# jhauret/vibravox

Hardware: AMD Instinct MI355X
Metric: EBEN train-step audio-seconds/sec (gen+disc) (higher is better)
Workload: dtype bf16

## Files before the change

### include/eben_hip.h

```cpp
#ifndef EBEN_HIP_H
#define EBEN_HIP_H

#include <stddef.h>
#include <stdint.h>

#if defined(EBEN_BUILDING)
#define EBEN_API __attribute__((visibility("default")))
#else
#define EBEN_API
#endif

#ifdef __cplusplus
extern "C" {
#endif

#define EBEN_OK 0
#define EBEN_EINVAL (-1)
#define EBEN_EWORKSPACE (-2)
#define EBEN_EUNSUPPORTED (-3)

#define EBEN_PAD_ZERO 0
#define EBEN_PAD_REFLECT 1

#define EBEN_MATH_F32 0
// ... 30 lines not shown
  int32_t rows, cols;
} EbenWnScaleItem;
typedef struct EbenWnBwdItem {
  const float* slabs;
  const float* g; const float* v; const float* norm;
  float* dg; float* dv; float* dbias;
  int64_t slab_stride;
  int32_t nslab, rows, cols, row_stride;
  int32_t col_perm_k, pad_;
} EbenWnBwdItem;
EBEN_API int eben_wn_scale_multi(const EbenWnScaleItem* items, int n, void* stream);
EBEN_API int eben_wn_bwd_multi(const EbenWnBwdItem* items, int n, void* stream);

EBEN_API size_t eben_conv1d_packed_floats(const EbenConv1dDesc* d, int which);
typedef struct EbenPackJob {
  EbenConv1dDesc desc;
  const float* v; const float* scale;
  float* wp_fwd; float* wp_bwd;
} EbenPackJob;
EBEN_API int eben_conv1d_pack_multi(const EbenPackJob* jobs, int n, void* stream);
#define EBEN_CONV_ROUTE_NONE 0
#define EBEN_CONV_ROUTE_TAP1 1
#define EBEN_CONV_ROUTE_TAP2 2
#define EBEN_CONV_ROUTE_THIN 3
#define EBEN_CONV_ROUTE_TAP3 4
#define EBEN_CONV_ROUTE_GC 5
#define EBEN_CONV_ROUTE_TAP4 6
EBEN_API int eben_conv1d_kernel_generation(const EbenConv1dDesc* d, int which);
#define EBEN_VARIANT_TAP3 1
#define EBEN_VARIANT_THIN_BL 2
#define EBEN_VARIANT_TAP4 3
#define EBEN_VARIANT_GC 4
EBEN_API int eben_conv1d_variant(const EbenConv1dDesc* d, int which, int mask_on_load, int* out, int n);
EBEN_API int eben_conv1d_variant_f32(const EbenConv1dDesc* d, int which, int mask_on_load, int* out, int n);
EBEN_API int eben_conv1d_pack(const EbenConv1dDesc* d, const float* v, const float* scale, float* wp_fwd, float* wp_bwd, void* stream);
EBEN_API int eben_conv1d_fwd(const EbenConv1dDesc* d, const float* x, const float* wp_fwd, const float* bias,
                    const float* residual, float* y, void* stream);
EBEN_API int eben_conv1d_fwd_res(const EbenConv1dDesc* d, const float* x, const float* wp_fwd, const float* bias,
                        const float* residual, float res_slope, float* y, void* stream);
EBEN_API size_t eben_conv1d_bwd_dx_workspace(const EbenConv1dDesc* d);
EBEN_API size_t eben_conv1d_bwd_dw_workspace(const EbenConv1dDesc* d, int* nslab, int* row_stride);
EBEN_API int eben_conv1d_bwd_dx(const EbenConv1dDesc* d, const float* dy, const float* y, const float* wp_bwd,
                       const float* x, float* dx, int accumulate, void* workspace, size_t ws_bytes, void* stream);
EBEN_API int eben_conv1d_bwd_dx_res(const EbenConv1dDesc* d, const float* dy, const float* y, const float* wp_bwd, const float* x,
                           const float* res_pre, const float* res_post, float* dx, void* workspace, size_t ws_bytes, void* stream);
EBEN_API int eben_conv1d_bwd_dx_ex(const EbenConv1dDesc* d, const float* g, const float* wp_bwd, const float* res, int res_rows,
                          const float* mask, float mask_slope, int seg, const int* seg_map, float* dx, void* stream);
EBEN_API int eben_conv1d_bwd_dx_fm(const EbenConv1dDesc* d, const float* g, const float* wp_bwd, const float* ref, int fm_rows,
                          const float* fm_sums, float fm_gs, const float* mask, float mask_slope, int seg, const int* seg_map,
                          float* dx, void* stream);
EBEN_API int eben_conv1d_bwd_dw(const EbenConv1dDesc* d, const float* dy, const float* y, const float* x, int has_bias,
                       float* slabs, size_t ws_bytes, void* stream);
#define EBEN_DW_ROUTE_TINY 0
#define EBEN_DW_ROUTE_ONE_ROW 1
#define EBEN_DW_ROUTE_DW3 2
#define EBEN_DW_ROUTE_DW2 3
#define EBEN_DW_ROUTE_FALLBACK 4
EBEN_API int eben_conv1d_bwd_dw_variant(const EbenConv1dDesc* d, int* out, int n);
EBEN_API int eben_conv1d_bwd_dw_f32_variant(const EbenConv1dDesc* d, int* out, int n);

EBEN_API int eben_bl_from_f32(const float* x, int batch, int channels, int length, void* hi, void* lo , void* stream);
EBEN_API int eben_bl_to_f32(const void* hi, const void* lo , int batch, int channels, int length, float* x, void* stream);
EBEN_API int eben_bl_conv1d_fwd(const EbenConv1dDesc* d, const void* x_hi, const void* x_lo, const float* wp_fwd, const float* bias,
                       void* y_hi, void* y_lo, void* stream);
EBEN_API int eben_bl_conv1d_bwd_dx(const EbenConv1dDesc* d, const void* g_hi, const float* wp_bwd, const void* act_hi, const void* act_lo,
                          float mask_slope, int seg, const int* seg_map, int fm_rows, int ref_row_offset, const float* fm_sums,
// ... 388 lines not shown
```

### vibravox_amd/_lib.py

```python
from __future__ import annotations

import ctypes
import os
from ctypes import POINTER, c_char_p, c_float, c_int, c_int32, c_int64, c_size_t, c_void_p
from typing import Optional

import torch

_HERE = os.path.dirname(os.path.abspath(__file__))
LIB_PATH = os.path.join(_HERE, "lib", "libeben_hip.so")


class EbenError(RuntimeError):
    pass


class EbenConv1dDesc(ctypes.Structure):
    _fields_ = [
        ("batch", c_int32),
        ("c_in", c_int32),
        ("c_out", c_int32),
        ("l_in", c_int32),
        ("l_out", c_int32),
        ("ksize", c_int32),
# ... 107 lines not shown
    _fields_ = [("band", c_void_p), ("first", c_void_p), ("orig", c_int32), ("nw", c_int32), ("width", c_int32), ("W", c_int32)]


class EbenResampleClip(ctypes.Structure):
    _fields_ = [("src_offset", c_int64), ("t_in", c_int32), ("band", c_int32), ("dst_row", c_int32), ("reserved", c_int32)]


class EbenVocoderClip(ctypes.Structure):
    _fields_ = [("rate", ctypes.c_double), ("frames_out", c_int32), ("col_out", c_int32)]


class EbenOlaClip(ctypes.Structure):
    _fields_ = [("dst_offset", c_int64), ("col", c_int32), ("frames_out", c_int32), ("len_stretch", c_int32), ("valid", c_int32)]


class EbenMaskClip(ctypes.Structure):
    _fields_ = [("row", c_int32), ("first", c_int32), ("count", c_int32)]


_P = c_void_p
_D = POINTER(EbenConv1dDesc)

SIGNATURES = {
    "eben_last_error": (c_char_p, []),
    "eben_version": (c_int, []),
    "eben_device_info": (c_int, [ctypes.c_char_p, c_size_t]),
    "eben_wn_scale": (c_int, [_P, _P, c_int, c_int, _P, _P, _P]),
    "eben_wn_bwd": (c_int, [_P, c_int, c_size_t, c_int, c_int, c_int, _P, _P, _P, _P, _P, _P, _P]),
    "eben_wn_scale_multi": (c_int, [POINTER(EbenWnScaleItem), c_int, _P]),
    "eben_wn_bwd_multi": (c_int, [POINTER(EbenWnBwdItem), c_int, _P]),
    "eben_conv1d_packed_floats": (c_size_t, [_D, c_int]),
    "eben_conv1d_kernel_generation": (c_int, [_D, c_int]),
    "eben_conv1d_variant": (c_int, [_D, c_int, c_int, POINTER(c_int), c_int]),
    "eben_conv1d_variant_f32": (c_int, [_D, c_int, c_int, POINTER(c_int), c_int]),
    "eben_conv1d_pack": (c_int, [_D, _P, _P, _P, _P, _P]),
    "eben_conv1d_pack_multi": (c_int, [POINTER(EbenPackJob), c_int, _P]),
    "eben_conv1d_fwd": (c_int, [_D, _P, _P, _P, _P, _P, _P]),
    "eben_conv1d_fwd_res": (c_int, [_D, _P, _P, _P, _P, c_float, _P, _P]),
    "eben_conv1d_bwd_dx_res": (c_int, [_D, _P, _P, _P, _P, _P, _P, _P, _P, c_size_t, _P]),
    "eben_conv1d_bwd_dx_workspace": (c_size_t, [_D]),
    "eben_conv1d_bwd_dw_workspace": (c_size_t, [_D, POINTER(c_int), POINTER(c_int)]),
    "eben_conv1d_bwd_dx": (c_int, [_D, _P, _P, _P, _P, _P, c_int, _P, c_size_t, _P]),
    "eben_conv1d_bwd_dx_ex": (c_int, [_D, _P, _P, _P, c_int, _P, c_float, c_int, POINTER(c_int), _P, _P]),
    "eben_conv1d_bwd_dx_fm": (c_int, [_D, _P, _P, _P, c_int, _P, c_float, _P, c_float, c_int, POINTER(c_int), _P, _P]),
    "eben_conv1d_bwd_dw": (c_int, [_D, _P, _P, _P, c_int, _P, c_size_t, _P]),
    "eben_conv1d_bwd_dw_variant": (c_int, [_D, POINTER(c_int), c_int]),
    "eben_conv1d_bwd_dw_f32_variant": (c_int, [_D, POINTER(c_int), c_int]),
    "eben_bl_from_f32": (c_int, [_P, c_int, c_int, c_int, _P, _P, _P]),
    "eben_bl_to_f32": (c_int, [_P, _P, c_int, c_int, c_int, _P, _P]),
    "eben_bl_conv1d_fwd": (c_int, [_D, _P, _P, _P, _P, _P, _P, _P]),
    "eben_bl_conv1d_bwd_dx": (c_int, [_D, _P, _P, _P, _P, c_float, c_int, POINTER(c_int), c_int, c_int, _P, c_float, _P, _P, _P]),
    "eben_bl_dx_pr_desc": (c_int, [_D, _D]),
    "eben_bl_dx_pr_weights": (c_int, [_D, _P, _P, _P, _P]),
    "eben_bl_conv1d_bwd_dx_pr": (c_int, [_D, _P, _P, _P, _P, c_float, c_int, POINTER(c_int), c_int, c_int, _P, c_float, _P, _P, _P]),
    "eben_bl_conv1d_bwd_dx_c": (c_int, [_D, _P, _P, _P, _P, _P, c_float, c_int, POINTER(c_int), c_int, c_int, _P, c_float, _P, _P, _P]),
    "eben_bl_conv1d_bwd_dx_pr_c": (c_int, [_D, _P, _P, _P, _P, _P, c_float, c_int, POINTER(c_int), c_int, c_int, _P, c_float, _P, _P, _P]),
    "eben_bl_conv1d_bwd_dw_workspace": (c_size_t, [_D, POINTER(c_int), POINTER(c_int), POINTER(c_int)]),
    "eben_bl_conv1d_bwd_dw": (c_int, [_D, _P, _P, c_int, _P, c_size_t, _P]),
    "eben_bl_conv1d_bwd_dw_multi": (c_int, [POINTER(_D), POINTER(_P), POINTER(_P), c_int, POINTER(_P), POINTER(c_size_t), c_int, _P]),
    "eben_bl_conv1d_bwd_dw_variant": (c_int, [_D, POINTER(c_int), c_int]),
    "eben_bl_head_fwd": (c_int, [POINTER(EbenBlHeadJob), c_int, c_int, _P]),
    "eben_bl_head_dx": (c_int, [POINTER(EbenBlHeadJob), c_int, c_int, _P, _P]),
    "eben_bl_head_dw_workspace": (c_size_t, [POINTER(EbenBlHeadJob), c_int, POINTER(c_int), POINTER(c_int)]),
    "eben_bl_head_dw": (c_int, [POINTER(EbenBlHeadJob), c_int, _P, c_size_t, _P]),
    "eben_bl_tail_fwd": (c_int, [_P, _P, c_int, c_int, c_int, c_int, c_int, _P, _P, _P, c_float, _P, _P]),
    "eben_bl_tail_dx": (c_int, [_P, c_int, c_int, c_int, c_int, c_int, _P, _P, _P, _P, c_float, c_int, POINTER(c_int), c_int, c_int, _P, c_float,
# ... 191 lines not shown
```

### vibravox_amd/csrc/conv1d.hip

```cpp
#include "common.h"
#include "tap3.h"

#include <cstdlib>

namespace eben {

int canon_from_desc(const EbenConv1dDesc* d, Canon* c) {
  EBEN_REQUIRE(d != nullptr, "null conv descriptor");
  EBEN_REQUIRE(d->batch > 0 && d->c_in > 0 && d->c_out > 0 && d->l_in > 0 && d->l_out > 0, "non-positive conv dims");
  EBEN_REQUIRE(d->ksize > 0 && d->stride > 0 && d->dilation > 0 && d->groups > 0, "non-positive conv params");
  EBEN_REQUIRE(d->c_in % d->groups == 0 && d->c_out % d->groups == 0, "channels not divisible by groups");
  EBEN_REQUIRE(d->stride <= 1024 && d->pad_l >= 0 && d->pad_r >= 0, "bad stride / padding");
  c->B = d->batch; c->k = d->ksize; c->s = d->stride; c->d = d->dilation; c->g = d->groups;
  c->pl = d->pad_l; c->pr = d->pad_r;
  const int math = d->math & ~EBEN_LAYOUT_BL;
  EBEN_REQUIRE(math >= EBEN_MATH_F32 && math <= EBEN_MATH_BF16X6, "unknown math mode %d", d->math);
  c->bl = (d->math & EBEN_LAYOUT_BL) != 0;
  EBEN_REQUIRE(!c->bl || math == EBEN_MATH_BF16 || math == EBEN_MATH_BF16X3, "the bundle layout carries EBEN_MATH_BF16 / EBEN_MATH_BF16X3 only");
  c->bf16 = math != EBEN_MATH_F32;
  c->np = math == EBEN_MATH_BF16X3 ? 2 : (math == EBEN_MATH_BF16X6 ? 3 : 1);
  c->xsplit_dir = math == EBEN_MATH_BF16X2 ? (d->transposed ? 1 : 0) : -1;
  if (!d->transposed) {
    c->Cin = d->c_in; c->Cout = d->c_out; c->Lin = d->l_in; c->Lout = d->l_out;
    c->reflect = d->pad_mode == EBEN_PAD_REFLECT;
// ... 87 lines not shown

extern "C" size_t eben_conv1d_packed_floats(const EbenConv1dDesc* d, int which) {
  Canon c;
  if (canon_from_desc(d, &c) != EBEN_OK) return 0;
  const ConvRoute r = conv_route(c, d->transposed, which);
  return kConvFamilies[r.family].packed_floats(c, r.dir);
}

extern "C" int eben_conv1d_kernel_generation(const EbenConv1dDesc* d, int which) {
  Canon c;
  if (canon_from_desc(d, &c) != EBEN_OK) return EBEN_CONV_ROUTE_NONE;
  return conv_route(c, d->transposed, which).reported();
}

extern "C" int eben_conv1d_variant(const EbenConv1dDesc* d, int which, int mask_on_load, int* out, int n) {
  EBEN_REQUIRE(out && n >= 8 && (which == 0 || which == 1), "eben_conv1d_variant: which 0 / 1 and 8 output slots");
  EBEN_REQUIRE(!mask_on_load || which == 1, "eben_conv1d_variant: the mask is applied on load by input gradients only");
  Canon c;
  const int rc = canon_from_desc(d, &c);
  if (rc) return rc;
  for (int i = 0; i < 8; ++i) out[i] = 0;
  const ConvRoute r = conv_route(c, d->transposed, which);
  out[0] = r.reported();
  if (r.family == EBEN_CONV_ROUTE_GC) {
    if (gc_variant(c, r.dir, &out[1], &out[2], &out[3], &out[4])) out[7] = EBEN_VARIANT_GC;
    return EBEN_OK;
  }
  if (r.family != EBEN_CONV_ROUTE_TAP3) return EBEN_OK;
  Tap3Call k{};
  k.bl = c.bl; k.in_mode = mask_on_load ? 1 : 0; k.reflect = r.reflect;
  Tap3Variant v;
  if (const int e = tap3_plan_variant(c, r.dir, k, &v)) return e;
  out[1] = v.FM; out[2] = v.XRB; out[3] = v.IM; out[4] = v.NPW; out[5] = v.NPX; out[6] = v.BL; out[7] = v.kernel;
  return EBEN_OK;
}

extern "C" int eben_conv1d_variant_f32(const EbenConv1dDesc* d, int which, int mask_on_load, int* out, int n) {
  EBEN_REQUIRE(out && n >= 8 && (which == 0 || which == 1), "eben_conv1d_variant_f32: which 0 / 1 and 8 output slots");
  EBEN_REQUIRE(!mask_on_load || which == 1, "eben_conv1d_variant_f32: the mask is applied on load by input gradients only");
  Canon c;
  const int rc = canon_from_desc(d, &c);
  if (rc) return rc;
  for (int i = 0; i < 8; ++i) out[i] = 0;
  const ConvRoute r = conv_route(c, d->transposed, which);
  out[0] = r.reported();
  if (r.family == EBEN_CONV_ROUTE_THIN) return thin_plan_variant(c, r.dir, &out[1]);
  if (r.family == EBEN_CONV_ROUTE_TAP2) return tap2_plan_variant(c, r.dir, mask_on_load ? 1 : 0, &out[1]);
  return EBEN_OK;
}

extern "C" int eben_conv1d_pack(const EbenConv1dDesc* d, const float* v, const float* scale, float* wp_fwd, float* wp_bwd, void* stream) {
  Canon c;
  int rc = canon_from_desc(d, &c);
  if (rc) return rc;
  EBEN_REQUIRE(v != nullptr, "null weight");
  for (int which = 0; which < 2; ++which) {
    float* dst = which == 0 ? wp_fwd : wp_bwd;
    if (!dst) continue;
    const ConvRoute r = conv_route(c, d->transposed, which);
    if ((rc = kConvFamilies[r.family].pack(c, r.dir, v, scale, dst, as_stream(stream)))) return rc;
  }
  return EBEN_OK;
}

extern "C" int eben_conv1d_pack_multi(const EbenPackJob* jobs, int n, void* stream) {
  EBEN_REQUIRE(n >= 0 && (n == 0 || jobs != nullptr), "bad pack job list");
// ... 226 lines not shown
```

### vibravox_amd/csrc/tap3.h

```cpp
#pragma once
#include "common.h"

namespace eben {

typedef unsigned u32x4 __attribute__((ext_vector_type(4)));

struct Tap3Args {
  const float* x; const float* xmask; const u32x4* wp; const int* tab;
  const float* bias; const float* res; const float* emask; float* y;
  int B, G, Cg, Mg, Cx, Cy, Lx, Ly;
  int S, OS, dstep, J0, mode, off0, nt, nph;
  int ps_pad, ps_k, ps_d, ps_kstep;
  int reflect, accumulate, in_mode;
  int res_rows, em_seg, em_map[4];
  const float* fm_sums; float fm_gs;
  float in_slope, out_slope, res_slope, emask_slope;
  int CI_T, CI_B, CP, ncc, PLEN, CSTRIDE, nxb;
  unsigned s_magic;
  int ntt, nmt, tab_phase;
  long long w_tile, w_phase;
  const u32x4* xh; const u32x4* xl;
  uint2* yh; uint2* yl;
  const uint2* eh; const uint2* el;
  const unsigned* ec;
  int CBx, CBy, bl_ref_off, bl_pad;
  int pr_S, pr_cbg, pr_Ly, pr_order;
  unsigned xq, xr;
  unsigned m_nph, m_ntt, m_B, m_nmt;
  int id_fast, pg_n;
  int big_XT, big_PPT, big_tiles;
  unsigned m_cstride, m_plen;
  struct PG { int J, off0, minoff, nt, oo, span; unsigned span_magic; int pad; } pg[8];
};

struct Tap3Plan {
  int ok;
  int mode, G, Cg, Mg, S, OS, dstep, kstep, nph, J, Lx, Ly, Cx, Cy, off0, nt, ps_pad;
  int FM, BM, BN, WCHU;
  int dense;
  int npw, npx, KSC;
  int CI_T, CI_B, CP, ncc, PLEN, CSTRIDE, nxbuf, XRB;
  int nmt, ntt, NCH, tab_phase;
  long long w_tile, w_phase, tab_off_floats;
  size_t packed_floats, lds_bytes;
  int big, WM, WN, TM, TN, RING, XT, PPT, xbuf_stride;
};

struct Tap3Call { int bl, in_mode, pr_S, pr_order, reflect, bias, res, eh, accumulate; };
inline Tap3Call tap3_call_of(const Tap3Args& a, int reflect) {
  return Tap3Call{a.xh != nullptr, a.in_mode, a.pr_S, a.pr_order, reflect, a.bias != nullptr, a.res != nullptr, a.eh != nullptr, a.accumulate};
}
struct Tap3Variant { int kernel, FM, XRB, IM, NPW, NPX, BL, thin; };
int tap3_variant(const Tap3Plan& p, const Tap3Call& k, Tap3Variant* v);
int tap3_plan_variant(const Canon& c, int dir, const Tap3Call& k, Tap3Variant* v);

int tap4_launch(const Tap3Plan& p, const Tap3Args& a, hipStream_t st);
int thin_bl_form(const Tap3Plan& p, const Tap3Call& k);
int thin_bl_launch(const Tap3Plan& p, const Tap3Args& a, int form, int nblocks, hipStream_t st);

}
```

### vibravox_amd/csrc/tapconv3.hip

```cpp
#include "common.h"
#include "tap3.h"

#include <cstdlib>

namespace eben {

typedef float f32x16 __attribute__((ext_vector_type(16)));
typedef float f32x2 __attribute__((ext_vector_type(2)));
typedef __bf16 bf16x8 __attribute__((ext_vector_type(8)));
typedef __bf16 bf16x2 __attribute__((ext_vector_type(2)));

__device__ __forceinline__ unsigned pack_bf16(float a, float b) {
  const f32x2 v = {a, b};
  return __builtin_bit_cast(unsigned, __builtin_convertvector(v, bf16x2));
}

#ifndef EBEN_T3_KSC
#define EBEN_T3_KSC 4
#endif
#ifndef EBEN_T3_DBG
#define EBEN_T3_DBG 0
#endif
#if EBEN_T3_DBG & 512
constexpr int T3_STAMP_ROWS = 65536;
// ... 1157 lines not shown
#pragma unroll 1
  while (j + 1 < T.n && blockIdx.x >= T.first[j + 1]) ++j;
  pack3_body(T.job[j], blockIdx.x - T.first[j], T.first[j + 1] - T.first[j]);
}

template <int FM, int XRB, bool IM, int NPW = 1, int NPX = 1, bool BL = false>
static int launch3_im(const Tap3Args& a, int nblocks, size_t lds, hipStream_t st) {
  static LdsAttrOnce attr_once;
  auto kern = tap3_kernel<FM, XRB, IM, NPW, NPX, BL>;
  {
    const hipError_t e = lds_attr_once(attr_once, reinterpret_cast<const void*>(kern));
    if (e != hipSuccess) return hip_fail(e, "hipFuncSetAttribute(tap3)");
  }
  hipLaunchKernelGGL(kern, dim3(nblocks), dim3(256), lds, st, a);
  EBEN_CHECK_LAUNCH("tap3_kernel");
  return EBEN_OK;
}
template <int FM, int XRB>
static int launch3_cfg(const Tap3Args& a, int nblocks, size_t lds, const Tap3Variant& v, hipStream_t st) {
  if (v.BL) return v.NPW == 2 ? launch3_im<FM, XRB, false, 2, 2, true>(a, nblocks, lds, st) : launch3_im<FM, XRB, false, 1, 1, true>(a, nblocks, lds, st);
  if (v.NPX > 1) {
    if (v.NPW == 1) return launch3_im<FM, XRB, false, 1, 2>(a, nblocks, lds, st);
    if (v.NPW == 2) return launch3_im<FM, XRB, false, 2, 2>(a, nblocks, lds, st);
    return launch3_im<FM, XRB, false, 3, 3>(a, nblocks, lds, st);
  }
  return v.IM ? launch3_im<FM, XRB, true>(a, nblocks, lds, st) : launch3_im<FM, XRB, false>(a, nblocks, lds, st);
}

int tap3_variant(const Tap3Plan& p, const Tap3Call& k, Tap3Variant* v) {
  *v = Tap3Variant{};
  if (!p.ok) return fail(EBEN_EUNSUPPORTED, "tap3_launch on a layer the bf16 kernel does not cover");
  if (k.bl && (k.in_mode || p.npw != p.npx || p.npw > 2))
    return fail(EBEN_EUNSUPPORTED, "tap3: bundle layout with %d / %d operand pieces or a mask on load", p.npw, p.npx);
  v->FM = p.FM; v->NPW = p.npw; v->NPX = p.npx; v->BL = k.bl ? 1 : 0;
  if (p.big) { v->kernel = EBEN_VARIANT_TAP4; return EBEN_OK; }
  if ((v->thin = thin_bl_form(p, k))) { v->kernel = EBEN_VARIANT_THIN_BL; return EBEN_OK; }
  v->kernel = EBEN_VARIANT_TAP3;
  v->XRB = p.XRB == 2 || p.XRB == 3 ? p.XRB : 5;
  if (!k.bl && p.npx > 1 && k.in_mode) return fail(EBEN_EUNSUPPORTED, "tap3: split operand with a mask on load");
  v->IM = !k.bl && p.npx == 1 && k.in_mode ? 1 : 0;
  return EBEN_OK;
}

int tap3_plan_variant(const Canon& c, int dir, const Tap3Call& k, Tap3Variant* v) {
  Tap3Plan p;
  make_plan3(c, dir, &p);
  return tap3_variant(p, k, v);
}

int tap3_applicable(const Canon& c, int dir) {
  Tap3Plan p;
  make_plan3(c, dir, &p);
  return p.ok;
}

int tap3_is_big(const Canon& c, int dir) {
  Tap3Plan p;
  make_plan3(c, dir, &p);
  return p.ok && p.big;
}

size_t tap3_packed_floats(const Canon& c, int dir) {
  Tap3Plan p;
  make_plan3(c, dir, &p);
  return p.ok ? p.packed_floats : 0;
}

// ... 186 lines not shown
```

### vibravox_amd/csrc/thin_bl.hip

```cpp
#include "common.h"
#include "tap3.h"

#include <cstdlib>

namespace eben {
namespace thin {

typedef float f32x16 __attribute__((ext_vector_type(16)));
typedef float f32x2 __attribute__((ext_vector_type(2)));
typedef __bf16 bf16x8 __attribute__((ext_vector_type(8)));
typedef __bf16 bf16x2 __attribute__((ext_vector_type(2)));

__device__ __forceinline__ unsigned pack_bf16(float a, float b) {
  const f32x2 v = {a, b};
  return __builtin_bit_cast(unsigned, __builtin_convertvector(v, bf16x2));
}
template <int N> __device__ __forceinline__ void wait_vm() {
  static_assert(N >= 0 && N < 64, "vmcnt is a 6-bit count");
  __builtin_amdgcn_s_waitcnt((N & 15) | ((N >> 4) << 14) | 0x70);
}
__device__ u32x4 zero_unit = {0u, 0u, 0u, 0u};

enum { FWD = 0, DX_PR = 1, DX_PS = 2 };

constexpr int ksc_of(int np) { return np == 1 ? 4 : 2; }
constexpr int RING = 2;

template <int FM, int NP, int DIR, int S>
__global__ __launch_bounds__(256, NP >= 2 ? 1 : 2) void thin_bl_kernel(const Tap3Args P) {
  constexpr int NT = 256, BN = 128, BM = FM * 32, KSC = ksc_of(NP);
  constexpr int WCHU = KSC * NP * FM * 64;
  constexpr int WU = (WCHU + NT - 1) / NT;
  constexpr int CS = DIR == FWD ? S : 1;
  constexpr bool DMA_X = CS == 1;
  constexpr bool DX = DIR != FWD;
  static_assert(WCHU % 64 == 0, "weight chunk must split into whole wave pieces");

  extern __shared__ __attribute__((aligned(16))) u32x4 smem_thin[];
  u32x4* Ws = smem_thin;
  u32x4* Xs = smem_thin + RING * WCHU;

  const int tid = threadIdx.x;
  const int lane = tid & 63;
  const int wn = __builtin_amdgcn_readfirstlane(tid >> 6);

  unsigned id;
  {
    const unsigned bid = blockIdx.x, xcd = bid & 7u, idx = bid >> 3;
    id = (xcd < P.xr ? xcd * (P.xq + 1) : P.xr * (P.xq + 1) + (xcd - P.xr) * P.xq) + idx;
  }
  int ph = 0, tt, b, mt, g;
  if (P.id_fast) {
    unsigned qd;
    if constexpr (DIR == DX_PS) { qd = P.m_nph ? __umulhi(id, P.m_nph) : id; ph = (int)(id - qd * (unsigned)P.nph); id = qd; }
    qd = P.m_ntt ? __umulhi(id, P.m_ntt) : id; tt = (int)(id - qd * (unsigned)P.ntt); id = qd;
    qd = P.m_B ? __umulhi(id, P.m_B) : id; b = (int)(id - qd * (unsigned)P.B); id = qd;
    qd = P.m_nmt ? __umulhi(id, P.m_nmt) : id; mt = (int)(id - qd * (unsigned)P.nmt); g = (int)qd;
  } else {
    if constexpr (DIR == DX_PS) { ph = id % P.nph; id /= P.nph; }
    tt = id % P.ntt; id /= P.ntt;
    b = id % P.B; id /= P.B;
    mt = id % P.nmt;
    g = id / P.nmt;
  }
  ph = __builtin_amdgcn_readfirstlane(ph); tt = __builtin_amdgcn_readfirstlane(tt); b = __builtin_amdgcn_readfirstlane(b);
  mt = __builtin_amdgcn_readfirstlane(mt); g = __builtin_amdgcn_readfirstlane(g);
  const int t0 = tt * BN, m0 = mt * BM;

  const int J = P.pg[ph].J, nt = P.pg[ph].nt, oo = DIR == DX_PS ? P.pg[ph].oo : 0, minoff = P.pg[ph].minoff, span = P.pg[ph].span;
  const unsigned span_magic = P.pg[ph].span_magic;
  if (t0 >= nt) return;
  const int KS = J * P.CP;
  const int nch = (KS + KSC - 1) / KSC;
  const int q0 = t0 * CS + minoff;
  const int xtot = P.CI_B * span;
  const int XBUF = P.CI_B * P.CSTRIDE;
  const int LOU = NP > 1 ? XBUF + 1 : 0;

  const u32x4* wsrc = P.wp + (long long)ph * P.w_phase + ((long long)g * P.nmt + mt) * P.w_tile;
  typedef const __attribute__((address_space(4))) int* ctab_t;
  ctab_t tab = (ctab_t)(P.tab + (long long)ph * P.tab_phase);

  f32x16 acc[FM];
#pragma unroll
  for (int i = 0; i < FM; ++i)
#pragma unroll
    for (int r = 0; r < 16; ++r) acc[i][r] = 0.f;

  const int CgB = P.Cg >> 3;
  const long long xrowB = ((long long)b * P.CBx + (long long)g * CgB) * P.Lx;
  const bool inside = q0 >= 0 && q0 + span <= P.Lx;

  auto issue_w = [&](int ch) {
    const u32x4* src = wsrc + (long long)ch * WCHU;
    u32x4* dst = Ws + (ch % RING) * WCHU;
#pragma unroll
    for (int u = 0; u < WU; ++u) {
      int idx = u * NT + tid;
      if (WCHU % NT != 0 && idx >= WCHU) idx -= NT;
      __builtin_amdgcn_global_load_lds((const __attribute__((address_space(1))) void*)(src + idx),
                                       (__attribute__((address_space(3))) void*)(dst + (idx & ~63)), 16, 0, 0);
    }
  };

  int eb = b;
  if constexpr (DX) {
    eb = P.em_seg > 0 ? P.em_map[(int)(b >= P.em_seg) + (int)(b >= 2 * P.em_seg) + (int)(b >= 3 * P.em_seg)] * P.em_seg +
                            (b - ((int)(b >= P.em_seg) + (int)(b >= 2 * P.em_seg) + (int)(b >= 3 * P.em_seg)) * P.em_seg) : b;
  }
  float* Bs = reinterpret_cast<float*>(Xs + NP * (XBUF + 1));
  float fk1 = 0.f, fk2 = 0.f;
  const bool fmr = DX && P.fm_sums != nullptr && P.res_rows > 0 && b < P.res_rows;
  if constexpr (!DX) {
    if (tid < BM) {
      const int m = m0 + tid;
      Bs[tid] = P.bias ? P.bias[(long long)g * P.Mg + (m < P.Mg ? m : P.Mg - 1)] : 0.f;
    }
  } else if (fmr) {
    typedef const __attribute__((address_space(4))) float* cf_t;
    const float s1 = ((cf_t)P.fm_sums)[0], s2 = ((cf_t)P.fm_sums)[1];
    fk1 = P.fm_gs / s2; fk2 = P.fm_gs * s1 / (s2 * s2);
  }
  if (nch > 0) {
    issue_w(0);
    if constexpr (DMA_X) {
      const int ppr = (span + 63) >> 6;
      int bb = 0, pr = __builtin_amdgcn_readfirstlane(tid >> 6);
      while (pr >= ppr) { pr -= ppr; ++bb; }
      while (bb < P.CI_B) {
        const int r = pr * 64 + lane;
        const int qq = q0 + r;
        const bool in = qq >= 0 && qq < P.Lx && bb < CgB;
        const long long idx = xrowB + (long long)(bb < CgB ? bb : 0) * P.Lx + (in ? qq : 0);
        u32x4* d = Xs + bb * P.CSTRIDE + pr * 64;
        if (r < span) {
          __builtin_amdgcn_global_load_lds((const __attribute__((address_space(1))) void*)(in ? P.xh + idx : &zero_unit),
                                           (__attribute__((address_space(3))) void*)d, 16, 0, 0);
          if constexpr (NP > 1)
            __builtin_amdgcn_global_load_lds((const __attribute__((address_space(1))) void*)(in ? P.xl + idx : &zero_unit),
                                             (__attribute__((address_space(3))) void*)(d + LOU), 16, 0, 0);
        }
        pr += NT / 64;
        while (pr >= ppr) { pr -= ppr; ++bb; }
      }
    } else {
      struct Round { u32x4 w[2][NP]; int sl[2], ok[2]; };
      auto pro_load = [&](int base, Round& R) {
#pragma unroll
        for (int u = 0; u < 2; ++u) {
          const int i = base + tid + u * NT;
          const int bb = (int)__umulhi((unsigned)i, span_magic);
          const int r = i - bb * span;
          int qq = q0 + (i < xtot ? r : 0), ok = 1;
          if (!inside) {
            ok = (int)(qq >= 0) & (int)(qq < P.Lx);
            qq = ok ? qq : 0;
          }
          ok &= (int)(i < xtot);
          const int c0 = i < xtot ? bb : 0;
          ok &= (int)(c0 < CgB);
          const long long idx = xrowB + (long long)(c0 < CgB ? c0 : 0) * P.Lx + qq;
          R.w[u][0] = P.xh[idx];
          if constexpr (NP > 1) R.w[u][1] = P.xl[idx];
          R.ok[u] = ok;
          const int d = r / CS, p = r - d * CS;
          R.sl[u] = i < xtot ? bb * P.CSTRIDE + p * P.PLEN + d : -1;
        }
      };
      auto pro_store = [&](Round& R) {
#pragma unroll
        for (int u = 0; u < 2; ++u)
          if (R.sl[u] >= 0) {
#pragma unroll
            for (int q = 0; q < NP; ++q) Xs[R.sl[u] + q * LOU] = R.ok[u] ? R.w[u][q] : u32x4{0u, 0u, 0u, 0u};
          }
      };
      Round ra, rb;
      if (xtot > 0) pro_load(0, ra);
      for (int base = 0; base < xtot; base += 4 * NT) {
        const bool second = base + 2 * NT < xtot;
        if (second) pro_load(base + 2 * NT, rb);
        pro_store(ra);
        if (second) {
          if (base + 4 * NT < xtot) pro_load(base + 4 * NT, ra);
          pro_store(rb);
        }
      }
    }
  }
  __syncthreads();
  constexpr bool PREF = DIR == DX_PS && FM <= 2;
  uint2 pah[PREF ? FM : 1][4];
  if constexpr (PREF) {
    if (P.eh != nullptr) {
      const int tq = t0 + wn * 32 + (lane & 31);
      const unsigned loffq = (((unsigned)(tq < nt ? tq : nt - 1) * (unsigned)P.OS + (unsigned)oo) * 2u + (unsigned)(lane >> 5)) * 8u;
      const long long Lrowq = (long long)P.Ly * 16;
      const char* ehq = reinterpret_cast<const char*>(P.eh) + (long long)eb * P.CBy * Lrowq + ((long long)((g * P.Mg + m0) >> 3)) * Lrowq;
      const int quadsq = (P.Mg - m0 + 7) >> 3;
#pragma unroll
      for (int i = 0; i < FM; ++i)
#pragma unroll
        for (int r4 = 0; r4 < 4; ++r4) {
          const int q = 4 * i + r4;
          pah[i][r4] = *reinterpret_cast<const uint2*>(ehq + (long long)(q < quadsq ? q : 0) * Lrowq + loffq);
        }
    }
  }

  const int lanebase = (lane >> 5) * P.CSTRIDE + wn * 32 + (lane & 31);
  int te[KSC];
#pragma unroll
  for (int ks = 0; ks < KSC; ++ks) te[ks] = nch > 0 ? tab[ks] : 0;
  constexpr int H = KSC >= 2 ? KSC / 2 : 1, H2 = KSC - H;
  u32x4 bvA[H][NP], aA[H][NP][FM], bvB[H2 > 0 ? H2 : 1][NP], aB[H2 > 0 ? H2 : 1][NP][FM];
  auto mma = [&](const u32x4 (&bq)[NP], const u32x4 (&aq)[NP][FM]) {
#pragma unroll
    for (int lvl = NP - 1; lvl >= 0; --lvl)
#pragma unroll
      for (int qw = 0; qw < NP; ++qw) {
        const int qx = lvl - qw;
        if (qx < 0 || qx >= NP) continue;
#pragma unroll
        for (int i = 0; i < FM; ++i)
          acc[i] = __builtin_amdgcn_mfma_f32_32x32x16_bf16(__builtin_bit_cast(bf16x8, aq[qw][i]), __builtin_bit_cast(bf16x8, bq[qx]), acc[i], 0, 0, 0);
      }
  };
  for (int ch = 0; ch < nch; ++ch) {
    int tn[KSC];
#pragma unroll
    for (int ks = 0; ks < KSC; ++ks) tn[ks] = tab[(ch + 1 < nch ? ch + 1 : ch) * KSC + ks];
    if (ch + 1 < nch) issue_w(ch + 1);
    const u32x4* wb = Ws + (ch % RING) * WCHU + lane;
    const u32x4* xb = Xs + lanebase;
    auto rd = [&](int ks, u32x4 (&bq)[NP], u32x4 (&aq)[NP][FM]) {
#pragma unroll
      for (int q = 0; q < NP; ++q) bq[q] = xb[te[ks] + q * LOU];
#pragma unroll
      for (int q = 0; q < NP; ++q)
#pragma unroll
        for (int i = 0; i < FM; ++i) aq[q][i] = wb[((ks * NP + q) * FM + i) * 64];
    };
#pragma unroll
    for (int h = 0; h < H; ++h) rd(h, bvA[h], aA[h]);
    __builtin_amdgcn_sched_barrier(0);
    if (ch > 0) {
#pragma unroll
      for (int h = 0; h < H2; ++h) mma(bvB[h], aB[h]);
    }
    __builtin_amdgcn_sched_barrier(0);
#pragma unroll
    for (int h = 0; h < H2; ++h) rd(H + h, bvB[h], aB[h]);
    __builtin_amdgcn_sched_barrier(0);
#pragma unroll
    for (int h = 0; h < H; ++h) mma(bvA[h], aA[h]);
    __builtin_amdgcn_sched_barrier(0);
#pragma unroll
    for (int ks = 0; ks < KSC; ++ks) te[ks] = tn[ks];
    wait_vm<0>();
    __builtin_amdgcn_s_barrier();
  }
  if (nch > 0) {
#pragma unroll
    for (int h = 0; h < H2; ++h) mma(bvB[h], aB[h]);
  }

  const int t = t0 + wn * 32 + (lane & 31);
  if (t >= nt) return;
  const int hb = lane >> 5;
  auto unpack = [](uint2 w, float (&f)[4]) {
    f[0] = __builtin_bit_cast(float, w.x << 16); f[1] = __builtin_bit_cast(float, w.x & 0xffff0000u);
    f[2] = __builtin_bit_cast(float, w.y << 16); f[3] = __builtin_bit_cast(float, w.y & 0xffff0000u);
  };
  const bool masked = DX && P.eh != nullptr;
  const bool fmc = fmr && masked && P.ec != nullptr;

  if constexpr (DIR == DX_PR) {
    constexpr bool s4 = S == 4;
    static_assert(S == 2 || S == 4, "phases as rows at stride 2 or 4");
    const int tile0i = m0 >> 5;
    const long long LrowP = (long long)P.pr_Ly * 16;
    const long long tileP = (long long)(g * P.pr_cbg) * LrowP;
    const char* ehp = reinterpret_cast<const char*>(P.eh) + (long long)eb * P.CBy * LrowP + tileP;
    const char* elp = reinterpret_cast<const char*>(P.el) + (long long)eb * P.CBy * LrowP + tileP;
    const char* rhp = reinterpret_cast<const char*>(P.eh) + (long long)(b + P.bl_ref_off) * P.CBy * LrowP + tileP;
    const char* rlp = reinterpret_cast<const char*>(P.el) + (long long)(b + P.bl_ref_off) * P.CBy * LrowP + tileP;
    char* yhp = reinterpret_cast<char*>(P.yh) + (long long)b * P.CBy * LrowP + tileP;
    char* ylp = reinterpret_cast<char*>(P.yl) + (long long)b * P.CBy * LrowP + tileP;
    const int pos0 = s4 ? 4 * t + 2 * hb : 2 * t;
    const bool lv0 = pos0 < P.pr_Ly, lv1 = pos0 + 1 < P.pr_Ly;
    const unsigned poff = (unsigned)(lv0 ? pos0 : 0) * 16u;
// ... 173 lines not shown
                v[e] += fk1 * (float)((int)(c & 3u) - 1) - fk2 * (float)((int)((c >> 2) & 3u) - 1);
              }
            } else if (fmr) {
              float a1[4], r0[4], r1[4];
              unpack(al[r4], a1); unpack(rh[r4], r0); unpack(rl[r4], r1);
#pragma unroll
              for (int e = 0; e < 4; ++e) {
                const float av = a0[e] + a1[e], dv = av - (r0[e] + r1[e]);
                v[e] += fk1 * (float)((dv > 0.f) - (dv < 0.f)) - fk2 * (float)((av > 0.f) - (av < 0.f));
              }
            }
#pragma unroll
            for (int e = 0; e < 4; ++e) v[e] *= dlrelu(a0[e], P.emask_slope);
          } else {
#pragma unroll
            for (int e = 0; e < 4; ++e) v[e] = lrelu(v[e], P.out_slope);
          }
          uint2 h;
          h.x = pack_bf16(v[0], v[1]); h.y = pack_bf16(v[2], v[3]);
          *reinterpret_cast<uint2*>(yhb + row + loff) = h;
          if (P.yl) {
            float hf[4];
            unpack(h, hf);
            uint2 l;
            l.x = pack_bf16(v[0] - hf[0], v[1] - hf[1]); l.y = pack_bf16(v[2] - hf[2], v[3] - hf[3]);
            *reinterpret_cast<uint2*>(ylb + row + loff) = l;
          }
        }
      }
    }
  }
}

template <int FM, int NP, int DIR, int S>
static int launch(const Tap3Args& a, int nblocks, size_t lds, hipStream_t st) {
  static LdsAttrOnce attr_once;
  auto kern = thin_bl_kernel<FM, NP, DIR, S>;
  {
    const hipError_t e = lds_attr_once(attr_once, reinterpret_cast<const void*>(kern));
    if (e != hipSuccess) return hip_fail(e, "hipFuncSetAttribute(thin_bl)");
  }
  hipLaunchKernelGGL(kern, dim3(nblocks), dim3(256), lds, st, a);
  EBEN_CHECK_LAUNCH("thin_bl_kernel");
  return EBEN_OK;
}

template <int NP, int DIR, int S>
static int launch_fm(int FM, const Tap3Args& a, int nblocks, size_t lds, hipStream_t st) {
  switch (FM) {
    case 1: return launch<1, NP, DIR, S>(a, nblocks, lds, st);
    case 2: return launch<2, NP, DIR, S>(a, nblocks, lds, st);
    case 3: return launch<3, NP, DIR, S>(a, nblocks, lds, st);
    default: return launch<4, NP, DIR, S>(a, nblocks, lds, st);
  }
}

enum { FORM_FWD_NP2_S2 = 1, FORM_FWD_NP1_S4, FORM_DX_PR_S2, FORM_DX_PR_S4, FORM_DX_PS };

}

int thin_bl_form(const Tap3Plan& p, const Tap3Call& k) {
  static const int enabled = getenv("EBEN_THIN_BL") ? atoi(getenv("EBEN_THIN_BL")) : 1;
  if (!enabled || !k.bl || p.big || k.reflect || k.in_mode || p.npw != p.npx || p.npw > 2) return 0;
  if (p.ncc != 1 || p.nxbuf != 1 || p.nph > 8 || p.FM < 1 || p.FM > 4 || p.BN != 128) return 0;
  if (p.KSC != thin::ksc_of(p.npw) || p.WCHU != p.KSC * p.npw * p.FM * 64) return 0;
  if (p.lds_bytes != (size_t)thin::RING * p.WCHU * 16 + ((size_t)p.CI_B * p.CSTRIDE * 16 + 16) * p.npx + (size_t)p.BM * 4) return 0;
  if (p.Cg > 128 || p.Mg > 256) return 0;
  if (p.mode == 0 && k.pr_S == 0) {
    if (k.eh || k.res || k.accumulate || p.nph != 1) return 0;
    if (p.S == 2 && p.npw == 2) return thin::FORM_FWD_NP2_S2;
    if (p.S == 4 && p.npw == 1) return thin::FORM_FWD_NP1_S4;
    return 0;
  }
  if (p.npw != 1 || k.bias || k.res || k.accumulate) return 0;
  if (p.mode == 0) {
    if (k.pr_order != 1 || p.S != 1 || p.nph != 1) return 0;
    if (k.pr_S == 2) return thin::FORM_DX_PR_S2;
    if (k.pr_S == 4) return thin::FORM_DX_PR_S4;
    return 0;
  }
  if (p.S != 1 || p.OS != 2 || p.nph != 2) return 0;
  return thin::FORM_DX_PS;
}

int thin_bl_launch(const Tap3Plan& p, const Tap3Args& a, int form, int nblocks, hipStream_t st) {
  const size_t lds = p.lds_bytes;
  switch (form) {
    case thin::FORM_FWD_NP2_S2: return thin::launch_fm<2, thin::FWD, 2>(p.FM, a, nblocks, lds, st);
    case thin::FORM_FWD_NP1_S4: return thin::launch_fm<1, thin::FWD, 4>(p.FM, a, nblocks, lds, st);
    case thin::FORM_DX_PR_S2: return thin::launch_fm<1, thin::DX_PR, 2>(p.FM, a, nblocks, lds, st);
    case thin::FORM_DX_PR_S4: return thin::launch_fm<1, thin::DX_PR, 4>(p.FM, a, nblocks, lds, st);
    case thin::FORM_DX_PS: return thin::launch_fm<1, thin::DX_PS, 1>(p.FM, a, nblocks, lds, st);
    default: return fail(EBEN_EINVAL, "thin_bl: no thin form %d", form);
  }
}

}
```

Measured before the change: 7614.

## Extend thin bundle-layout conv kernel to multi-chunk input channels with double-buffered X

```diff
diff --git a/include/eben_hip.h b/include/eben_hip.h
--- a/include/eben_hip.h
+++ b/include/eben_hip.h
@@ -86,6 +86,7 @@
 #define EBEN_VARIANT_TAP4 3
 #define EBEN_VARIANT_GC 4
 EBEN_API int eben_conv1d_variant(const EbenConv1dDesc* d, int which, int mask_on_load, int* out, int n);
+EBEN_API int eben_bl_conv1d_thin_form(const EbenConv1dDesc* d, int which, int* out, int n);
 EBEN_API int eben_conv1d_variant_f32(const EbenConv1dDesc* d, int which, int mask_on_load, int* out, int n);
 EBEN_API int eben_conv1d_pack(const EbenConv1dDesc* d, const float* v, const float* scale, float* wp_fwd, float* wp_bwd, void* stream);
 EBEN_API int eben_conv1d_fwd(const EbenConv1dDesc* d, const float* x, const float* wp_fwd, const float* bias,
diff --git a/vibravox_amd/_lib.py b/vibravox_amd/_lib.py
--- a/vibravox_amd/_lib.py
+++ b/vibravox_amd/_lib.py
@@ -163,6 +163,7 @@
     "eben_conv1d_packed_floats": (c_size_t, [_D, c_int]),
     "eben_conv1d_kernel_generation": (c_int, [_D, c_int]),
     "eben_conv1d_variant": (c_int, [_D, c_int, c_int, POINTER(c_int), c_int]),
+    "eben_bl_conv1d_thin_form": (c_int, [_D, c_int, POINTER(c_int), c_int]),
     "eben_conv1d_variant_f32": (c_int, [_D, c_int, c_int, POINTER(c_int), c_int]),
     "eben_conv1d_pack": (c_int, [_D, _P, _P, _P, _P, _P]),
     "eben_conv1d_pack_multi": (c_int, [POINTER(EbenPackJob), c_int, _P]),
diff --git a/vibravox_amd/csrc/conv1d.hip b/vibravox_amd/csrc/conv1d.hip
--- a/vibravox_amd/csrc/conv1d.hip
+++ b/vibravox_amd/csrc/conv1d.hip
@@ -143,6 +143,31 @@
   Tap3Variant v;
   if (const int e = tap3_plan_variant(c, r.dir, k, &v)) return e;
   out[1] = v.FM; out[2] = v.XRB; out[3] = v.IM; out[4] = v.NPW; out[5] = v.NPX; out[6] = v.BL; out[7] = v.kernel;
+  return EBEN_OK;
+}
+
+extern "C" int eben_bl_conv1d_thin_form(const EbenConv1dDesc* d, int which, int* out, int n) {
+  EBEN_REQUIRE(out && n >= 4 && which >= 0 && which <= 2, "eben_bl_conv1d_thin_form: which 0 / 1 / 2 and 4 output slots");
+  Canon c, q;
+  const int rc = canon_from_desc(d, &c);
+  if (rc) return rc;
+  EBEN_REQUIRE(c.bl && !d->transposed, "eben_bl_conv1d_thin_form: a Conv1d descriptor with EBEN_LAYOUT_BL");
+  for (int i = 0; i < 4; ++i) out[i] = 0;
+  Tap3Call k{};
+  k.bl = 1;
+  Tap3Variant v;
+  if (which == 2) {
+    const PrGeom g = pr_geometry(c, &q);
+    if (!g.ok) return fail(EBEN_EUNSUPPORTED, "eben_bl_conv1d_thin_form: the layer's input gradient has no phases-as-rows form");
+    k.pr_S = g.S; k.pr_order = g.order; k.eh = 1;
+    if (const int e = tap3_plan_variant(q, 0, k, &v)) return e;
+  } else {
+    const ConvRoute r = conv_route(c, 0, which);
+    if (r.family != EBEN_CONV_ROUTE_TAP3) return EBEN_OK;
+    k.reflect = r.reflect; k.bias = which == 0; k.eh = which == 1;
+    if (const int e = tap3_plan_variant(c, r.dir, k, &v)) return e;
+  }
+  out[0] = v.thin; out[1] = v.FM; out[2] = v.ncc; out[3] = v.nxbuf;
   return EBEN_OK;
 }
 
diff --git a/vibravox_amd/csrc/tap3.h b/vibravox_amd/csrc/tap3.h
--- a/vibravox_amd/csrc/tap3.h
+++ b/vibravox_amd/csrc/tap3.h
@@ -50,7 +50,7 @@
 inline Tap3Call tap3_call_of(const Tap3Args& a, int reflect) {
   return Tap3Call{a.xh != nullptr, a.in_mode, a.pr_S, a.pr_order, reflect, a.bias != nullptr, a.res != nullptr, a.eh != nullptr, a.accumulate};
 }
-struct Tap3Variant { int kernel, FM, XRB, IM, NPW, NPX, BL, thin; };
+struct Tap3Variant { int kernel, FM, XRB, IM, NPW, NPX, BL, thin, ncc, nxbuf; };
 int tap3_variant(const Tap3Plan& p, const Tap3Call& k, Tap3Variant* v);
 int tap3_plan_variant(const Canon& c, int dir, const Tap3Call& k, Tap3Variant* v);
 
diff --git a/vibravox_amd/csrc/tapconv3.hip b/vibravox_amd/csrc/tapconv3.hip
--- a/vibravox_amd/csrc/tapconv3.hip
+++ b/vibravox_amd/csrc/tapconv3.hip
@@ -1213,7 +1213,7 @@
   if (!p.ok) return fail(EBEN_EUNSUPPORTED, "tap3_launch on a layer the bf16 kernel does not cover");
   if (k.bl && (k.in_mode || p.npw != p.npx || p.npw > 2))
     return fail(EBEN_EUNSUPPORTED, "tap3: bundle layout with %d / %d operand pieces or a mask on load", p.npw, p.npx);
-  v->FM = p.FM; v->NPW = p.npw; v->NPX = p.npx; v->BL = k.bl ? 1 : 0;
+  v->FM = p.FM; v->NPW = p.npw; v->NPX = p.npx; v->BL = k.bl ? 1 : 0; v->ncc = p.ncc; v->nxbuf = p.nxbuf;
   if (p.big) { v->kernel = EBEN_VARIANT_TAP4; return EBEN_OK; }
   if ((v->thin = thin_bl_form(p, k))) { v->kernel = EBEN_VARIANT_THIN_BL; return EBEN_OK; }
   v->kernel = EBEN_VARIANT_TAP3;
diff --git a/vibravox_amd/csrc/thin_bl.hip b/vibravox_amd/csrc/thin_bl.hip
--- a/vibravox_amd/csrc/thin_bl.hip
+++ b/vibravox_amd/csrc/thin_bl.hip
@@ -21,13 +21,17 @@
 }
 __device__ u32x4 zero_unit = {0u, 0u, 0u, 0u};
 
-enum { FWD = 0, DX_PR = 1, DX_PS = 2 };
+enum { FWD = 0, DX_PR = 1, DX_PS = 2, FWD_MC = 3, DX_PR_MC = 4 };
 
 constexpr int ksc_of(int np) { return np == 1 ? 4 : 2; }
 constexpr int RING = 2;
 
-template <int FM, int NP, int DIR, int S>
+template <int FM, int NP, int FORM, int S>
 __global__ __launch_bounds__(256, NP >= 2 ? 1 : 2) void thin_bl_kernel(const Tap3Args P) {
+  constexpr bool MC = FORM >= FWD_MC;
+  constexpr int DIR = MC ? FORM - FWD_MC : FORM;
+  constexpr int NXB = MC ? 2 : 1;
+  constexpr int XRB = 3;
   constexpr int NT = 256, BN = 128, BM = FM * 32, KSC = ksc_of(NP);
   constexpr int WCHU = KSC * NP * FM * 64;
   constexpr int WU = (WCHU + NT - 1) / NT;
@@ -70,12 +74,13 @@
   const int J = P.pg[ph].J, nt = P.pg[ph].nt, oo = DIR == DX_PS ? P.pg[ph].oo : 0, minoff = P.pg[ph].minoff, span = P.pg[ph].span;
   const unsigned span_magic = P.pg[ph].span_magic;
   if (t0 >= nt) return;
-  const int KS = J * P.CP;
+  const int KS_CC = J * P.CP;
+  const int KS = MC ? P.ncc * KS_CC : KS_CC;
   const int nch = (KS + KSC - 1) / KSC;
   const int q0 = t0 * CS + minoff;
   const int xtot = P.CI_B * span;
   const int XBUF = P.CI_B * P.CSTRIDE;
-  const int LOU = NP > 1 ? XBUF + 1 : 0;
+  const int LOU = NP > 1 ? NXB * XBUF + 1 : 0;
 
   const u32x4* wsrc = P.wp + (long long)ph * P.w_phase + ((long long)g * P.nmt + mt) * P.w_tile;
   typedef const __attribute__((address_space(4))) int* ctab_t;
@@ -103,12 +108,76 @@
     }
   };
 
+  auto dma_tile = [&](int cc, u32x4* dst) {
+    const int ppr = (span + 63) >> 6;
+    int bb = 0, pr = __builtin_amdgcn_readfirstlane(tid >> 6);
+    while (pr >= ppr) { pr -= ppr; ++bb; }
+    while (bb < P.CI_B) {
+      const int r = pr * 64 + lane;
+      const int qq = q0 + r;
+      const int cbn = cc * P.CI_B + bb;
+      const bool in = qq >= 0 && qq < P.Lx && cbn < CgB;
+      const long long idx = xrowB + (long long)(cbn < CgB ? cbn : 0) * P.Lx + (in ? qq : 0);
+      u32x4* d = dst + bb * P.CSTRIDE + pr * 64;
+      if (r < span) {
+        __builtin_amdgcn_global_load_lds((const __attribute__((address_space(1))) void*)(in ? P.xh + idx : &zero_unit),
+                                         (__attribute__((address_space(3))) void*)d, 16, 0, 0);
+        if constexpr (NP > 1)
+          __builtin_amdgcn_global_load_lds((const __attribute__((address_space(1))) void*)(in ? P.xl + idx : &zero_unit),
+                                           (__attribute__((address_space(3))) void*)(d + LOU), 16, 0, 0);
+      }
+      pr += NT / 64;
+      while (pr >= ppr) { pr -= ppr; ++bb; }
+    }
+  };
+  constexpr bool RS_MC = MC && !DMA_X;
+  int xsl[RS_MC ? XRB : 1], xbb[RS_MC ? XRB : 1], xqq[RS_MC ? XRB : 1];
+  unsigned xinb = 0, okmask = 0;
+  u32x4 xru[RS_MC ? XRB : 1][NP];
+  if constexpr (RS_MC) {
+#pragma unroll
+    for (int u = 0; u < XRB; ++u) {
+      const int i = tid + u * NT;
+      const int bb = (int)__umulhi((unsigned)i, span_magic);
+      const int r = i - bb * span;
+      const int qq = q0 + (i < xtot ? r : 0);
+      const int in = inside ? 1 : ((int)(qq >= 0) & (int)(qq < P.Lx));
+      xinb |= (unsigned)(in & (int)(i < xtot)) << u;
+      xqq[u] = in ? qq : 0;
+      xbb[u] = i < xtot ? bb : 0;
+      const int d = r / CS, p = r - d * CS;
+      xsl[u] = i < xtot ? bb * P.CSTRIDE + p * P.PLEN + d : -1;
+    }
+  }
+  auto fetch_x = [&](int cc) {
+    okmask = 0;
+#pragma unroll
+    for (int u = 0; u < (RS_MC ? XRB : 0); ++u) {
+      const int cbn = cc * P.CI_B + xbb[u];
+      const bool cin = cbn < CgB;
+      okmask |= (((xinb >> u) & 1u) & (unsigned)cin) << u;
+      const long long idx = xrowB + (long long)(cin ? cbn : 0) * P.Lx + xqq[u];
+      xru[u][0] = P.xh[idx];
+      if constexpr (NP > 1) xru[u][1] = P.xl[idx];
+    }
+  };
+  auto store_x = [&](int cc) {
+    u32x4* dst = Xs + (cc & 1) * XBUF;
+#pragma unroll
+    for (int u = 0; u < (RS_MC ? XRB : 0); ++u)
+      if (xsl[u] >= 0) {
+        const bool live = (okmask >> u) & 1u;
+#pragma unroll
+        for (int q = 0; q < NP; ++q) dst[xsl[u] + q * LOU] = live ? xru[u][q] : u32x4{0u, 0u, 0u, 0u};
+      }
+  };
+
   int eb = b;
   if constexpr (DX) {
     eb = P.em_seg > 0 ? P.em_map[(int)(b >= P.em_seg) + (int)(b >= 2 * P.em_seg) + (int)(b >= 3 * P.em_seg)] * P.em_seg +
                             (b - ((int)(b >= P.em_seg) + (int)(b >= 2 * P.em_seg) + (int)(b >= 3 * P.em_seg)) * P.em_seg) : b;
   }
-  float* Bs = reinterpret_cast<float*>(Xs + NP * (XBUF + 1));
+  float* Bs = reinterpret_cast<float*>(Xs + NP * (NXB * XBUF + 1));
   float fk1 = 0.f, fk2 = 0.f;
   const bool fmr = DX && P.fm_sums != nullptr && P.res_rows > 0 && b < P.res_rows;
   if constexpr (!DX) {
@@ -123,7 +192,9 @@
   }
   if (nch > 0) {
     issue_w(0);
-    if constexpr (DMA_X) {
+    if constexpr (DMA_X && MC) {
+      dma_tile(0, Xs);
+    } else if constexpr (DMA_X) {
       const int ppr = (span + 63) >> 6;
       int bb = 0, pr = __builtin_amdgcn_readfirstlane(tid >> 6);
       while (pr >= ppr) { pr -= ppr; ++bb; }
@@ -186,6 +257,9 @@
           pro_store(rb);
         }
       }
+      if constexpr (MC) {
+        if (P.ncc > 1) fetch_x(1);
+      }
     }
   }
   __syncthreads();
@@ -226,11 +300,20 @@
           acc[i] = __builtin_amdgcn_mfma_f32_32x32x16_bf16(__builtin_bit_cast(bf16x8, aq[qw][i]), __builtin_bit_cast(bf16x8, bq[qx]), acc[i], 0, 0, 0);
       }
   };
+  int written = 0, pending = -1;
   for (int ch = 0; ch < nch; ++ch) {
     int tn[KSC];
 #pragma unroll
     for (int ks = 0; ks < KSC; ++ks) tn[ks] = tab[(ch + 1 < nch ? ch + 1 : ch) * KSC + ks];
     if (ch + 1 < nch) issue_w(ch + 1);
+    if constexpr (MC && DMA_X) {
+      if (written + 1 < P.ncc && (written + 1) * KS_CC < (ch + 2) * KSC) {
+        ++written;
+        dma_tile(written, Xs + (written & 1) * XBUF);
+      }
+    } else if constexpr (MC) {
+      if (pending >= 0) { fetch_x(pending); pending = -1; }
+    }
     const u32x4* wb = Ws + (ch % RING) * WCHU + lane;
     const u32x4* xb = Xs + lanebase;
     auto rd = [&](int ks, u32x4 (&bq)[NP], u32x4 (&aq)[NP][FM]) {
@@ -257,6 +340,13 @@
     __builtin_amdgcn_sched_barrier(0);
 #pragma unroll
     for (int ks = 0; ks < KSC; ++ks) te[ks] = tn[ks];
+    if constexpr (RS_MC) {
+      if (written + 1 < P.ncc && (written + 1) * KS_CC < (ch + 2) * KSC) {
+        ++written;
+        store_x(written);
+        if (written + 1 < P.ncc) pending = written + 1;
+      }
+    }
     wait_vm<0>();
     __builtin_amdgcn_s_barrier();
   }
@@ -496,10 +586,10 @@
   }
 }
 
-template <int FM, int NP, int DIR, int S>
+template <int FM, int NP, int FORM, int S>
 static int launch(const Tap3Args& a, int nblocks, size_t lds, hipStream_t st) {
   static LdsAttrOnce attr_once;
-  auto kern = thin_bl_kernel<FM, NP, DIR, S>;
+  auto kern = thin_bl_kernel<FM, NP, FORM, S>;
   {
     const hipError_t e = lds_attr_once(attr_once, reinterpret_cast<const void*>(kern));
     if (e != hipSuccess) return hip_fail(e, "hipFuncSetAttribute(thin_bl)");
@@ -519,31 +609,39 @@
   }
 }
 
-enum { FORM_FWD_NP2_S2 = 1, FORM_FWD_NP1_S4, FORM_DX_PR_S2, FORM_DX_PR_S4, FORM_DX_PS };
+enum { FORM_FWD_NP2_S2 = 1, FORM_FWD_NP1_S4, FORM_DX_PR_S2, FORM_DX_PR_S4, FORM_DX_PS, FORM_FWD_NP2_S2_MC, FORM_DX_PR_S2_MC };
 
 }
 
 int thin_bl_form(const Tap3Plan& p, const Tap3Call& k) {
   static const int enabled = getenv("EBEN_THIN_BL") ? atoi(getenv("EBEN_THIN_BL")) : 1;
+  static const int chunks = getenv("EBEN_THIN_BL_CHUNKS") ? atoi(getenv("EBEN_THIN_BL_CHUNKS")) : 1;
   if (!enabled || !k.bl || p.big || k.reflect || k.in_mode || p.npw != p.npx || p.npw > 2) return 0;
-  if (p.ncc != 1 || p.nxbuf != 1 || p.nph > 8 || p.FM < 1 || p.FM > 4 || p.BN != 128) return 0;
+  if (p.nph > 8 || p.FM < 1 || p.FM > 4 || p.BN != 128) return 0;
   if (p.KSC != thin::ksc_of(p.npw) || p.WCHU != p.KSC * p.npw * p.FM * 64) return 0;
-  if (p.lds_bytes != (size_t)thin::RING * p.WCHU * 16 + ((size_t)p.CI_B * p.CSTRIDE * 16 + 16) * p.npx + (size_t)p.BM * 4) return 0;
+  if (p.lds_bytes != (size_t)thin::RING * p.WCHU * 16 + ((size_t)p.nxbuf * p.CI_B * p.CSTRIDE * 16 + 16) * p.npx + (size_t)p.BM * 4) return 0;
+  const bool mc = p.ncc > 1;
+  if (mc) {
+    if (!chunks || p.nxbuf != 2 || p.FM != 3 || p.nph != 1 || p.NCH < 6) return 0;
+    if (p.J * p.CP < 2 * p.KSC || p.XRB < 2 || p.XRB > 3 || p.xbuf_stride != p.CI_B * p.CSTRIDE) return 0;
+  } else if (p.nxbuf != 1) {
+    return 0;
+  }
   if (p.Cg > 128 || p.Mg > 256) return 0;
   if (p.mode == 0 && k.pr_S == 0) {
     if (k.eh || k.res || k.accumulate || p.nph != 1) return 0;
-    if (p.S == 2 && p.npw == 2) return thin::FORM_FWD_NP2_S2;
-    if (p.S == 4 && p.npw == 1) return thin::FORM_FWD_NP1_S4;
+    if (p.S == 2 && p.npw == 2) return mc ? thin::FORM_FWD_NP2_S2_MC : thin::FORM_FWD_NP2_S2;
+    if (p.S == 4 && p.npw == 1 && !mc) return thin::FORM_FWD_NP1_S4;
     return 0;
   }
   if (p.npw != 1 || k.bias || k.res || k.accumulate) return 0;
   if (p.mode == 0) {
     if (k.pr_order != 1 || p.S != 1 || p.nph != 1) return 0;
-    if (k.pr_S == 2) return thin::FORM_DX_PR_S2;
-    if (k.pr_S == 4) return thin::FORM_DX_PR_S4;
+    if (k.pr_S == 2) return mc ? thin::FORM_DX_PR_S2_MC : thin::FORM_DX_PR_S2;
+    if (k.pr_S == 4 && !mc) return thin::FORM_DX_PR_S4;
     return 0;
   }
-  if (p.S != 1 || p.OS != 2 || p.nph != 2) return 0;
+  if (mc || p.S != 1 || p.OS != 2 || p.nph != 2) return 0;
   return thin::FORM_DX_PS;
 }
 
@@ -555,6 +653,8 @@
     case thin::FORM_DX_PR_S2: return thin::launch_fm<1, thin::DX_PR, 2>(p.FM, a, nblocks, lds, st);
     case thin::FORM_DX_PR_S4: return thin::launch_fm<1, thin::DX_PR, 4>(p.FM, a, nblocks, lds, st);
     case thin::FORM_DX_PS: return thin::launch_fm<1, thin::DX_PS, 1>(p.FM, a, nblocks, lds, st);
+    case thin::FORM_FWD_NP2_S2_MC: return thin::launch<3, 2, thin::FWD_MC, 2>(a, nblocks, lds, st);
+    case thin::FORM_DX_PR_S2_MC: return thin::launch<3, 1, thin::DX_PR_MC, 2>(a, nblocks, lds, st);
     default: return fail(EBEN_EINVAL, "thin_bl: no thin form %d", form);
   }
 }
```

Result: no change. 7579 (-0.5%).
